# Rouslan/NTracer

Measured on AMD Instinct MI355X. Metric: Mrays/s (primary+shadow), 6-D hypercube @1920x1080, higher is better.
Workload: dtype f32

## Files before the change

### ntracer_amd/build.py

```python
import concurrent.futures
import hashlib
import os
import shutil
import subprocess
import sys

HERE = os.path.dirname(os.path.abspath(__file__))
CSRC = os.path.join(HERE, "csrc")
OBJ = os.path.join(HERE, "build")
OUT = os.path.join(HERE, "libntracer_hip.so")
DIMS = range(3, 11)
BOX_ONLY_DIMS = range(11, 25)
HDR = [os.path.join(CSRC, h) for h in ("nt_device.hpp", "nt_pixel.hpp", "nt_box.hpp", "nt_composite.hpp", "nt_resolve.hpp", "nt_query.hpp", "nt_hits.hpp", "nt_rays.hpp", "nt_lens.hpp", "nt_parallel.hpp", "nt_adaptive.hpp", "nt_ao.hpp", "nt_outline.hpp", "nt_cue.hpp", "nt_clip.hpp", "nt_boxhits.hpp", "nt_dispatch.hpp")] + \
      [os.path.join(HERE, "..", "include", "ntracer_hip.h")]
FLAGS = ["--offload-arch=gfx950", "-O3", "-std=c++17", "-ffp-contract=off", "-fPIC", "-pthread", "-fno-slp-vectorize", "-Wall",
         "-Wno-unused-function"]
EXTRA = os.environ.get("NTRACER_HIPCC_FLAGS", "").split()


def units():
    u = [("nt_api", "nt_api.cpp", []), ("nt_builder", "nt_builder.cpp", []), ("nt_launch", "nt_launch.cpp", []),
         ("nt_var", "nt_var.hip", [])]
    for n in DIMS:
        u.append(("nt_box_%d" % n, "nt_inst_box.hip", ["-DNT_INST_N=%d" % n]))
        u.append(("nt_composite_%d" % n, "nt_inst_composite.hip", ["-DNT_INST_N=%d" % n]))
        u.append(("nt_query_%d" % n, "nt_inst_query.hip", ["-DNT_INST_N=%d" % n]))
        u.append(("nt_hits_%d" % n, "nt_inst_hits.hip", ["-DNT_INST_N=%d" % n]))
        u.append(("nt_rays_%d" % n, "nt_inst_rays.hip", ["-DNT_INST_N=%d" % n]))
        u.append(("nt_adaptive_%d" % n, "nt_inst_adaptive.hip", ["-DNT_INST_N=%d" % n]))
        u.append(("nt_lens_%d" % n, "nt_inst_lens.hip", ["-DNT_INST_N=%d" % n]))
        u.append(("nt_parallel_%d" % n, "nt_inst_parallel.hip", ["-DNT_INST_N=%d" % n]))
        u.append(("nt_ao_%d" % n, "nt_inst_ao.hip", ["-DNT_INST_N=%d" % n]))
        u.append(("nt_outline_%d" % n, "nt_inst_outline.hip", ["-DNT_INST_N=%d" % n]))
        u.append(("nt_cue_%d" % n, "nt_inst_cue.hip", ["-DNT_INST_N=%d" % n]))
        u.append(("nt_boxhits_%d" % n, "nt_inst_boxhits.hip", ["-DNT_INST_N=%d" % n]))
        u.append(("nt_clip_%d" % n, "nt_inst_clip.hip", ["-DNT_INST_N=%d" % n]))
    for n in BOX_ONLY_DIMS:
        u.append(("nt_box_%d" % n, "nt_inst_box.hip", ["-DNT_INST_N=%d" % n]))
        u.append(("nt_rays_%d" % n, "nt_inst_rays.hip", ["-DNT_INST_N=%d" % n]))
        u.append(("nt_adaptive_%d" % n, "nt_inst_adaptive.hip", ["-DNT_INST_N=%d" % n]))
        u.append(("nt_boxhits_%d" % n, "nt_inst_boxhits.hip", ["-DNT_INST_N=%d" % n]))
    return u


def hipcc():
    for c in (os.environ.get("HIPCC"), shutil.which("hipcc"), "/opt/rocm/bin/hipcc"):
# ... 77 lines not shown
```

### ntracer_amd/csrc/nt_api.cpp

```cpp
#include <hip/hip_runtime_api.h>

#include <algorithm>
#include <atomic>
#include <climits>
#include <cmath>
#include <cstdarg>
#include <cstdio>
#include <cstring>
#include <cstdlib>
#include <map>
#include <memory>
#include <mutex>
#include <new>
#include <string>
#include <thread>
#include <vector>

#include "../../include/ntracer_hip.h"
#include "nt_device.hpp"

namespace {

thread_local std::string g_error;

int fail(int code, const char *fmt, ...) {
    char buf[512];
    va_list ap;
    va_start(ap, fmt);
    vsnprintf(buf, sizeof(buf), fmt, ap);
    va_end(ap);
    g_error = buf;
    return code;
}

#define HIP_TRY(expr)                                                                          \
    do {                                                                                       \
        hipError_t e_ = (expr);                                                                \
        if (e_ != hipSuccess) return fail(e_ == hipErrorOutOfMemory ? NT_E_NOMEM : NT_E_DEVICE, \
                                          "%s failed: %s", #expr, hipGetErrorString(e_));       \
    } while (0)

struct DevBuf {
    void *p = nullptr;
    size_t cap = 0;
    int ensure(size_t bytes) {
        if (bytes <= cap && p) return 0;
        if (p) { (void)hipFree(p); p = nullptr; cap = 0; }
        size_t want = std::max<size_t>(bytes, 256);
        HIP_TRY(hipMalloc(&p, want));
        cap = want;
        return 0;
    }
// ... 527 lines not shown
    }
    return NT_OK;
}

struct RenderGuard {
    nt_scene *s;
    bool held = false;
    explicit RenderGuard(nt_scene *sc) : s(sc) {}
    int acquire() {
        std::lock_guard<std::mutex> g(s->mu);
        if (s->busy) return fail(NT_E_BUSY, "the renderer is already running");
        s->busy = true;
        ++s->locked;
        held = true;
        return NT_OK;
    }
    ~RenderGuard() {
        if (held) {
            std::lock_guard<std::mutex> g(s->mu);
            s->busy = false;
            --s->locked;
        }
    }
};

struct FrameJob {
    const Format *fmt;
    Bands bands;
    void *dest_dev;
    size_t frame_stride;
    int nframes;
    const float *cam_buf;
    const float *cam_dots = nullptr;
    hipStream_t stream;
    bool stats;
    bool strict = false;
    const int *abort_word = nullptr;
    int overlapped = 0;
    bool counters_pass = false;
    bool samples_pass = false;
    int row_begin, row_count;
    float *colors_out = nullptr;
    const int *xs = nullptr, *ys = nullptr;
    int probe_count = 0;
    int view_w = 0, view_h = 0;
};

struct RenderSwitches {
    bool strict_reference, clean_normals, force_var, numerators, two_pass, tile_order, box_cull, box_interleave, box_var_rows;
    int composite_kernel, frame_major, chunk_frames;
};

int atoi_or(const char *e, int unset) { return e ? atoi(e) : unset; }

RenderSwitches read_switches() {
    RenderSwitches sw;
    sw.strict_reference = atoi_or(getenv("NTRACER_STRICT_REFERENCE"), 0) != 0;
    sw.clean_normals = atoi_or(getenv("NTRACER_CLEAN_NORMALS"), 0) != 0;
    sw.force_var = atoi_or(getenv("NTRACER_FORCE_VAR"), 0) != 0;
    sw.composite_kernel = atoi_or(getenv("NTRACER_COMPOSITE_KERNEL"), 0);
    sw.numerators = atoi_or(getenv("NTRACER_NUMERATORS"), 1) != 0;
    sw.two_pass = atoi_or(getenv("NTRACER_TWO_PASS"), 1) != 0;
    sw.tile_order = atoi_or(getenv("NTRACER_TILE_ORDER"), 1) != 0;
    sw.frame_major = atoi_or(getenv("NTRACER_FRAME_MAJOR"), 1);
    sw.chunk_frames = atoi_or(getenv("NTRACER_CHUNK_FRAMES"), INT_MAX);
    sw.box_cull = atoi_or(getenv("NTRACER_BOX_CULL"), 1) != 0;
// ... 52 lines not shown
    return NT_OK;
}

int plain_f32_format(int w, int h, Format &out) {
    static const nt_channel plain[3] = {{1.0f, 0.0f, 0.0f, 0.0f, 32, 1, {0, 0}}, {0.0f, 1.0f, 0.0f, 0.0f, 32, 1, {0, 0}}, {0.0f, 0.0f, 1.0f, 0.0f, 32, 1, {0, 0}}};
    const nt_image_format desc = {(int32_t)w, (int32_t)h, 0, 3, plain, 0};
    return parse_format(&desc, out);
}

void view_target(const nt_scene *s, int w, int h, const int *abort_word, NtTarget &tg) {
    std::memset(&tg, 0, sizeof(tg));
    fill_view(tg, s, w, h);
    tg.band_world = 1;
    tg.band_rows = NT_RENDER_CHUNK_SIZE;
    tg.row_count = h;
    tg.abort_word = abort_word;
}

FrameJob base_frame_job(const nt_scene *s, const FrameJob &job, const Format &bf, int f0, int nf, void *dest, size_t frame_bytes) {
    FrameJob bj = job;
    bj.samples_pass = true;
    bj.fmt = &bf;
    bj.bands = Bands();
    bj.bands.owned_rows = bf.height;
    bj.row_begin = 0;
    bj.row_count = bf.height;
    bj.nframes = nf;
    bj.frame_stride = frame_bytes;
    bj.dest_dev = dest;
    bj.stats = false;
    if (job.cam_buf) {
        bj.cam_buf = job.cam_buf + (size_t)f0 * 4 * s->n;
        bj.cam_dots = job.cam_dots + (size_t)f0 * 4;
    }
    return bj;
}

int checked_scratch(const nt_scene *s, DeviceState *ds, const RenderSwitches &sw, NtCompositeDev &c, long long lanes_per_block, long long &blocks,
                    long long min_blocks, int frame_stack, long long cap_bytes) {
    const long long words = ((long long)s->n_batches + s->n_triangles + s->n_solids + 31) / 32;
    const long long fwords = (long long)nt_var_frame_words(s->n) * frame_stack;
    while (blocks > min_blocks && blocks * lanes_per_block * (words + fwords) * 4 > cap_bytes) blocks /= 2;
    if (int e = ds->checked.ensure((size_t)(blocks * lanes_per_block * words * 4))) return e;
    c.checked = (uint32_t *)ds->checked.p;
    c.checked_words = (int)words;
    c.checked_lanes = (int)(blocks * lanes_per_block);
    c.alias_normals = sw.clean_normals ? 0 : 1;
    if (frame_stack > 0) {
        if (int e = ds->tframes.ensure((size_t)(blocks * lanes_per_block * fwords * 4))) return e;
        c.tframes = (float *)ds->tframes.p;
        c.tframe_count = frame_stack;
    }
    return NT_OK;
}

int numerator_scratch(const nt_scene *s, DeviceState *ds, const RenderSwitches &sw, int nframes, NtLaunchInfo &li) {
    if (s->n_batches <= 0 || !sw.numerators) return NT_OK;
    const size_t per_frame = (size_t)s->n_batches * NT_BATCH_SIZE * sizeof(float);
    const size_t frames = std::max<size_t>(1, std::min<size_t>((size_t)nframes, ((size_t)256 << 20) / per_frame));
    if (int e = ds->numer.ensure(frames * per_frame)) return e;
    li.numer_buf = (float *)ds->numer.p;
    li.numer_frames = std::max(1, std::min((int)frames, sw.chunk_frames));
    return NT_OK;
}

int hit_record_scratch(DeviceState *ds, const RenderSwitches &sw, size_t per_frame, int nframes, NtLaunchInfo &li) {
// ... 162 lines not shown
    const long long row_bytes = hi_pitch * ss;
    if (hi_pitch > INT_MAX || hi_h > INT_MAX)
        return fail(NT_E_UNSUPPORTED, "supersampling %d of a %d x %d image: the %lld x %lld samples are beyond the 2^31 - 1 bytes a sample row "
                    "and the 2^31 - 1 sample rows the kernels address", ss, f.width, f.height, hi_w, hi_h);
    if (row_bytes > cap)
        return fail(NT_E_UNSUPPORTED, "supersampling %d of a %d pixel wide image: the samples of one row (%lld bytes) do not fit the scratch "
                    "buffer of %lld MiB (nt_scene_set_supersampling_scratch_mb)", ss, f.width, row_bytes, cap >> 20);
    Format hf;
    if (int r = plain_f32_format((int)hi_w, (int)hi_h, hf)) return r;
    const long long rows_fit = std::min<long long>(cap / row_bytes, 16384);
    const int chunk_rows = (int)std::min<long long>(rows_fit, job.row_count);
    const int chunk_frames = chunk_rows < job.row_count ? 1 : (int)std::max<long long>(1, std::min<long long>(job.nframes, cap / (row_bytes * chunk_rows)));
    if (int e = ds->samples.ensure((size_t)chunk_frames * chunk_rows * row_bytes)) return e;
    NtTarget tg;
    if (int r = fill_target(s, ds, job, tg)) return r;
    for (int f0 = 0; f0 < job.nframes; f0 += chunk_frames) {
        const int nf = std::min(chunk_frames, job.nframes - f0);
        for (int r0 = 0; r0 < job.row_count; r0 += chunk_rows) {
            const int rc = std::min(chunk_rows, job.row_count - r0);
            FrameJob hj = job;
            hj.samples_pass = true;
            hj.fmt = &hf;
            hj.bands.rows = ss * job.bands.rows;
            hj.bands.compact = 1;
            hj.bands.owned_rows = ss * job.bands.owned_rows;
            hj.row_begin = ss * (job.row_begin + r0);
            hj.row_count = ss * rc;
            hj.nframes = nf;
            hj.frame_stride = (size_t)(rc * row_bytes);
            hj.dest_dev = (char *)ds->samples.p - (long long)hj.row_begin * hi_pitch;
            if (job.cam_buf) {
                hj.cam_buf = job.cam_buf + (size_t)f0 * 4 * s->n;
                hj.cam_dots = job.cam_dots + (size_t)f0 * 4;
            }
            if (int e = enqueue(s, ds, hj)) return e;
            NtTarget rt = tg;
            rt.dest = tg.dest + (long long)f0 * tg.frame_stride;
            rt.row_begin = job.row_begin + r0;
            rt.row_count = rc;
            if (int r = nt_launch_resolve(ss, job.stream, ds->samples.p, (long long)hj.frame_stride, hi_pitch, nf, rt)) return launch_failed(r);
        }
    }
    return NT_OK;
}

int rays_scene(const nt_scene *s, DeviceState *ds, const RenderSwitches &sw, bool strict, long long count, long long lpb_fixed, long long max_fixed,
               NtCompositeDev &c);

int adaptive_check(const nt_scene *s, const Bands &b, bool stats) {
    if (!s->adaptive || s->supersampling <= 1) return NT_OK;
    if (b.world > 1) return fail(NT_E_UNSUPPORTED, "row bands (band_world %d) are not available with adaptive supersampling: a pixel's contrast needs its neighbours", b.world);
    if (stats) return fail(NT_E_UNSUPPORTED, "collect_stats is not available with adaptive supersampling");
    return NT_OK;
}

int enqueue_adaptive(nt_scene *s, DeviceState *ds, const FrameJob &job, const RenderSwitches &sw, uint8_t *mask_dev, bool mask_scratch,
                     uint8_t **mask_out) {
    const bool draw = job.fmt != nullptr;
    const int ss = s->supersampling;
    const int W = draw ? job.fmt->width : job.view_w, H = draw ? job.fmt->height : job.view_h;
    if (job.bands.world > 1) return fail(NT_E_UNSUPPORTED, "row bands (band_world %d) are not available with adaptive supersampling: a pixel's contrast needs its neighbours", job.bands.world);
    if (job.stats) return fail(NT_E_UNSUPPORTED, "collect_stats is not available with adaptive supersampling");
    if (draw && (job.row_begin != 0 || job.row_count != H)) return fail(NT_E_UNSUPPORTED, "a row range is not available with adaptive supersampling");
    if (draw && job.fmt->bpp == 0) return NT_OK;
    const long long px = (long long)W * H;
    const long long cap = (long long)s->ss_scratch_mb << 20;
// ... 672 lines not shown
    if (s->outlines && s->composite && !job.colors_out && !job.samples_pass && !job.counters_pass)
        return enqueue_outlines(s, ds, job, sw, nullptr, false, nullptr);
    if (s->ao_count > 0 && s->composite && !job.colors_out && !job.samples_pass && !job.counters_pass)
        return enqueue_ao(s, ds, job, sw, nullptr, nullptr);
    if (s->box_lines && !s->composite && !job.colors_out && !job.samples_pass && !job.counters_pass)
        return enqueue_box_lines(s, ds, job, sw, nullptr, false, nullptr);
    if (s->lens) return enqueue_lens(s, ds, job, sw);
    if (s->parallel > 0.0f) return enqueue_parallel(s, ds, job, sw);
    if (s->supersampling > 1 && s->adaptive && !job.colors_out && !job.samples_pass && !job.counters_pass)
        return enqueue_adaptive(s, ds, job, sw, nullptr, false, nullptr);
    if (s->supersampling > 1 && !job.colors_out && !job.samples_pass && !job.counters_pass) return enqueue_supersampled(s, ds, job);
    if (s->composite && job.stats && !job.counters_pass && !job.colors_out) {
        if (s->n > NT_MAX_FIXED_DIM) return fail(NT_E_UNSUPPORTED, "collect_stats is not available above %d dimensions (the run-time-n kernels keep no counters)", NT_MAX_FIXED_DIM);
        if (!s->all_opaque)
            return fail(NT_E_UNSUPPORTED, "collect_stats is not available for scenes with transparent materials (their kernels keep no counters)");
        if (s->n_solids > 0 && !sw.clean_normals) {
            const size_t bytes = (size_t)job.fmt->pitch * (size_t)(job.bands.compact ? job.bands.owned_rows : job.fmt->height);
            if (int e = ds->stats_frame.ensure(std::max<size_t>(bytes, 16))) return e;
            FrameJob cj = job;
            cj.counters_pass = true;
            cj.dest_dev = ds->stats_frame.p;
            cj.frame_stride = 0;
            if (job.nframes > 1) return fail(NT_E_UNSUPPORTED, "collect_stats on a multi-frame launch is not available for scenes with Solids");
            if (int e = enqueue(s, ds, cj)) return e;
            job.stats = false;
        }
    }
    NtTarget tg;
    if (int r = fill_target(s, ds, job, tg)) return r;
    if (!job.colors_out && (tg.row_count <= 0 || tg.bpp == 0)) return NT_OK;
    NtCamera cam;
    cam.buf = job.cam_buf;
    cam.dots = job.cam_dots;
    cam.n = s->n;
    if (!job.cam_buf) pack_camera(s->n, s->origin.data(), s->axes.data(), cam.inl);
    camera_dots(s->n, s->origin.data(), s->axes.data(), cam.odots);
    NtLaunchInfo li = launch_info(s, ds, sw, job.nframes, job.stream);
    int r;
    if (s->composite) {
        NtCompositeDev c;
        if (int e = plan_composite(s, ds, job, sw, tg, cam, li, c)) return e;
        r = nt_launch_composite(li, cam, c, tg);
    } else {
        if (int e = plan_box(s, ds, job, sw, tg, li)) return e;
        r = nt_launch_box(li, cam, tg);
    }
    if (r) return launch_failed(r);
    return NT_OK;
}

int prepare_stats(DeviceState *ds, hipStream_t st, bool on) {
    if (!on) return NT_OK;
    if (int r = ds->stats.ensure(8 * sizeof(unsigned long long))) return r;
    HIP_TRY(hipMemsetAsync(ds->stats.p, 0, 8 * sizeof(unsigned long long), st));
    return NT_OK;
}

int render_checks(const nt_scene *s, const Format &f, const Bands &b, bool stats) {
    if (int r = clip_check(s, b, stats, 0, b.owned_rows, f.height)) return r;
    if (int r = cue_check(s, b, stats, 0, b.owned_rows, f.height)) return r;
    if (int r = outline_check(s, b, stats, 0, b.owned_rows, f.height)) return r;
    if (int r = ao_check(s, b, stats, 0, b.owned_rows, f.height)) return r;
    if (int r = box_lines_check(s, b, stats, 0, b.owned_rows, f.height)) return r;
    if (int r = lens_check(s, f.width, f.height, b, stats, false)) return r;
    if (int r = parallel_check(s, b, stats, false)) return r;
    return adaptive_check(s, b, stats);
// ... 1167 lines not shown
    }
    if (int r = use_stream(ds, (hipStream_t)hip_stream)) return r;
    const int n = s->n;
    const size_t cam_floats = (size_t)nframes * 4 * n + (size_t)nframes * 4;
    DeviceState::Stage *st = nullptr;
    if (int r = stage_slot(ds, cam_floats * sizeof(float), st)) return r;
    float *packed = (float *)st->host;
    pack_cameras(n, nframes, origins, axes, packed);
    if (int r = ds->cams.ensure(cam_floats * sizeof(float))) return r;
    if (int r = nt_launch_upload(hip_stream, packed, (float *)ds->cams.p, (int)cam_floats)) return launch_failed(r);
    HIP_TRY(hipEventRecord(st->done, (hipStream_t)hip_stream));
    st->in_flight = true;
    if (int r = prepare_stats(ds, (hipStream_t)hip_stream, stats)) return r;
    if (stats) { s->have_stats = false; s->stats_device = ds->device; }
    FrameJob job = render_job(f, b, dest_dev, frame_stride, nframes, (hipStream_t)hip_stream, stats, opts, true);
    job.cam_buf = (const float *)ds->cams.p;
    job.cam_dots = job.cam_buf + (size_t)nframes * 4 * s->n;
    return enqueue(s, ds, job);
}

struct nt_camera_table {
    int n = 0, nframes = 0, device = -1;
    float *dev = nullptr;
};

nt_camera_table_t *nt_camera_table_create(int dimension, int nframes, const float *origins, const float *axes, int device) {
    if (dimension < 3 || dimension > NT_MAX_DIM || nframes < 1 || nframes > 65535 || !origins || !axes) {
        fail(NT_E_INVALID, "invalid camera table arguments");
        return nullptr;
    }
    int dev;
    if (pick_device(nullptr, device, dev)) return nullptr;
    const int n = dimension;
    const size_t cam_floats = (size_t)nframes * 4 * n + (size_t)nframes * 4;
    std::vector<float> packed(cam_floats);
    pack_cameras(n, nframes, origins, axes, packed.data());
    void *p = nullptr;
    if (hipMalloc(&p, cam_floats * sizeof(float)) != hipSuccess) { fail(NT_E_NOMEM, "hipMalloc failed for the camera table"); return nullptr; }
    if (hipMemcpy(p, packed.data(), cam_floats * sizeof(float), hipMemcpyHostToDevice) != hipSuccess) {
        (void)hipFree(p);
        fail(NT_E_DEVICE, "camera table upload failed");
        return nullptr;
    }
    nt_camera_table *t = new (std::nothrow) nt_camera_table();
    if (!t) { (void)hipFree(p); fail(NT_E_NOMEM, "out of memory"); return nullptr; }
    t->n = n; t->nframes = nframes; t->device = dev; t->dev = (float *)p;
    return t;
}

void nt_camera_table_destroy(nt_camera_table_t *t) {
    if (!t) return;
    if (t->dev && hipSetDevice(t->device) == hipSuccess) { (void)hipDeviceSynchronize(); (void)hipFree(t->dev); }
    delete t;
}

int nt_camera_table_frames(const nt_camera_table_t *t) { return t ? t->nframes : fail(NT_E_INVALID, "table is NULL"); }

int nt_render_table_device(nt_scene_t *s, void *dest_dev, size_t frame_stride, const nt_camera_table_t *table, int first, int count,
                           const nt_image_format *fmt, const nt_render_opts *opts, void *hip_stream) {
    if (!s || !dest_dev || !table) return fail(NT_E_INVALID, "NULL argument");
    if (table->n != s->n) return fail(NT_E_INVALID, "the camera table is for %d dimensions, the scene has %d", table->n, s->n);
    if (first < 0 || count < 1 || first > table->nframes - count) return fail(NT_E_INVALID, "frames %d..%d are not in a table of %d", first, first + count - 1, table->nframes);
    Format f;
    if (int r = parse_format(fmt, f)) return r;
    Bands b;
    if (int r = parse_bands(opts, f.height, b)) return r;
    if (frame_stride < required_len(f, b)) return fail(NT_E_INVALID, "frame_stride is smaller than one frame");
    if (int r = check_renderable(s)) return r;
    std::lock_guard<std::mutex> g(s->mu);
    if (s->busy) return fail(NT_E_BUSY, "the renderer is already running");
    const bool stats = opts && opts->collect_stats;
    if (int r = render_checks(s, f, b, stats)) return r;
    DeviceState *ds;
    if (int r = scene_on_device(s, opts, -1, ds, table->device, "render")) return r;
    if (int r = use_stream(ds, (hipStream_t)hip_stream)) return r;
    if (int r = prepare_stats(ds, (hipStream_t)hip_stream, stats)) return r;
    if (stats) { s->have_stats = false; s->stats_device = ds->device; }
    FrameJob job = render_job(f, b, dest_dev, frame_stride, count, (hipStream_t)hip_stream, stats, opts, true);
    job.cam_buf = table->dev + (size_t)first * 4 * table->n;
    job.cam_dots = table->dev + (size_t)table->nframes * 4 * table->n + (size_t)first * 4;
    return enqueue(s, ds, job);
}

namespace {
int mask_validate(const nt_scene *s, int width, int height, const void *mask, const nt_render_opts *opts) {
    if (!s || !mask) return fail(NT_E_INVALID, "NULL argument");
    if (width < 1 || height < 1) return fail(NT_E_INVALID, "invalid view size");
    if (int r = clip_refuses(s, "the adaptive mask")) return r;
    if (!s->adaptive) return fail(NT_E_INVALID, "the adaptive threshold is off (nt_scene_set_adaptive_supersampling)");
    if (opts && opts->band_world > 1)
        return fail(NT_E_UNSUPPORTED, "the adaptive mask is of the whole image: row bands (band_world %d) are not available", opts->band_world);
    if (opts && opts->collect_stats) return fail(NT_E_UNSUPPORTED, "the adaptive mask keeps no counters: collect_stats is not available");
    if (s->lens || s->parallel > 0.0f) return fail(NT_E_UNSUPPORTED, "the adaptive mask is not available while a lens or the parallel projection is set");
    return check_renderable(s);
}
}

int nt_adaptive_mask(nt_scene_t *s, int width, int height, uint8_t *mask, long long *flagged, const nt_render_opts *opts) {
    if (int r = mask_validate(s, width, height, mask, opts)) return r;
    RenderGuard guard(s);
    if (int r = guard.acquire()) return r;
    DeviceState *ds;
    if (int r = scene_on_device(s, opts, -1, ds)) return r;
    if (int r = use_own_stream(ds)) return r;
    const FrameJob job = view_job(width, height, ds->stream, opts, false);
    uint8_t *mask_dev = nullptr;
    if (int r = enqueue_adaptive(s, ds, job, read_switches(), nullptr, true, &mask_dev)) { (void)hipStreamSynchronize(ds->stream); return r; }
    int count = 0;
    HIP_TRY(hipMemcpyAsync(mask, mask_dev, (size_t)width * height, hipMemcpyDeviceToHost, ds->stream));
    HIP_TRY(hipMemcpyAsync(&count, ds->refine_count.p, sizeof(int), hipMemcpyDeviceToHost, ds->stream));
    HIP_TRY(hipStreamSynchronize(ds->stream));
    if (flagged) *flagged = count;
    return NT_OK;
// ... 317 lines not shown
```

### ntracer_amd/csrc/nt_box.hpp

```cpp
#pragma once
#include <type_traits>
#include "nt_pixel.hpp"

namespace {

__device__ __forceinline__ bool box_may_hit(int n, const float *dots, float sx, float sy, float sq) {
    const float osq = dots[0];
    const float ov = fmaf(-dots[2], sy, fmaf(dots[1], sx, dots[3]));
    const float rad2 = (float)n * (1.0f + NT_FUZZ) * (1.0f + NT_FUZZ) * 1.001f;
#ifdef NT_EXP_SKIP_SLABS
    return false;
#else
    return !((osq - rad2) * sq > ov * ov * 1.0001f);
#endif
}

__device__ __forceinline__ void box_background(float in, float &r, float &g, float &b) {
    if (in > 0.0f) { r = in; g = in; b = in; }
    else { r = 0.0f; g = -in; b = -in; }
}

template <int N>
__device__ __forceinline__ void box_color(const float (&o)[N], const float (&dir)[N], bool maybe, float &r, float &g, float &b) {
    bool done = false;
    float shade = 0.0f;

    {
        float num[N];
        bool pre[N];
        float aK = 0.0f, bK = 1.0f, oK = 0.0f;
        bool any = false;
#pragma unroll
        for (int i = 0; i < N; ++i) {
            const float di = dir[i];
            const float s = di < 0.0f ? 1.0f : -1.0f;
// ... 13 lines not shown
                bool ok = tie && dist > 0.0f;
#pragma unroll
                for (int j = 0; j < N; ++j) {
                    if (j != i) {
                        const float p = dir[j] * dist + o[j];
                        ok = ok && !(fabsf(p) > (1.0f + NT_FUZZ));
                    }
                }
                if (ok) {
                    done = true;
                    if (dist >= FLT_MAX) shade = -1.0f;
                    else {
                        const float sine = di * (di < 0.0f ? 1.0f : -1.0f);
                        shade = sine <= 0.0f ? -sine : 0.0f;
                    }
                }
            }
        }
    }
    if (done && shade >= 0.0f) {
        r = shade * 1.0f;
        g = shade * 0.5f;
        b = shade * 0.5f;
    } else {
        box_background(dir[0], r, g, b);
    }
}

#ifndef NT_BOX_INLINE_MAX_N
#define NT_BOX_INLINE_MAX_N 8
#endif
#ifndef NT_BOX_SETS_MAX_N
#define NT_BOX_SETS_MAX_N NT_BOX_INLINE_MAX_N
#endif
#ifndef NT_BOX_MARGIN
#define NT_BOX_MARGIN 1e-5f
#endif
template <int N>
__device__ __forceinline__ void box_classify(const float (&o)[N], const float (&v)[N], float m, bool maybe, bool &hit, bool &unclear,
                                             float &x, float (&near)[N], float &tn, float &vK) {
    float tn2 = -INFINITY;
    tn = -INFINITY;
    vK = 0.0f;
    float tnp = -INFINITY, tfp = INFINITY;
    const float m1p = 1.0f + m;
#pragma unroll
    for (int j = 0; j < N; ++j) {
        const float inv = __builtin_amdgcn_rcpf(v[j]);
        const float c0 = -o[j] * inv;
        const float nr = c0 - fabsf(inv);
        near[j] = nr;
        tnp = fmaxf(tnp, fmaf(-fabsf(inv), m1p, c0));
        tfp = fminf(tfp, fmaf(fabsf(inv), m1p, c0));
        const bool later = nr > tn;
        tn2 = __builtin_amdgcn_fmed3f(tn, tn2, nr);
        vK = later ? v[j] : vK;
        tn = fmaxf(tn, nr);
    }
    const bool miss = tnp > tfp || tfp < 0.0f;
    const float c = 1.0f - m;
    float sum = 0.0f;
#pragma unroll
    for (int j = 0; j < N; ++j) sum = sum + fmaxf(fabsf(fmaf(v[j], tn, o[j])), c);
    const bool inside = sum - (float)N * c <= 1.5f * m;
    const bool sole = (tn - tn2) * fabsf(vK) > m;
    const bool front = tn > 1e-3f && tn < 1e30f;
    hit = maybe && !miss && inside && sole && front;
    unclear = maybe && !miss && !hit;
#ifdef NT_EXP_NOUNCLEAR
    unclear = false;
#endif
    x = hit ? vK : v[0];
}

__device__ __forceinline__ float nt_vmax(float a, float b) { float r; asm("v_max_f32 %0, %1, %2" : "=v"(r) : "v"(a), "v"(b)); return r; }
__device__ __forceinline__ float nt_vmin(float a, float b) { float r; asm("v_min_f32 %0, %1, %2" : "=v"(r) : "v"(a), "v"(b)); return r; }
__device__ __forceinline__ float nt_vmax3(float a, float b, float c) { float r; asm("v_max3_f32 %0, %1, %2, %3" : "=v"(r) : "v"(a), "v"(b), "v"(c)); return r; }
__device__ __forceinline__ float nt_vmin3(float a, float b, float c) { float r; asm("v_min3_f32 %0, %1, %2, %3" : "=v"(r) : "v"(a), "v"(b), "v"(c)); return r; }
__device__ __forceinline__ float nt_vmed3(float a, float b, float c) { float r; asm("v_med3_f32 %0, %1, %2, %3" : "=v"(r) : "v"(a), "v"(b), "v"(c)); return r; }
__device__ __forceinline__ float nt_vmax_abs(float a, float b) { float r; asm("v_max_f32 %0, |%1|, %2" : "=v"(r) : "v"(a), "v"(b)); return r; }
__device__ __forceinline__ float nt_vmax3_abs(float a, float b, float c) { float r; asm("v_max3_f32 %0, %1, |%2|, |%3|" : "=v"(r) : "v"(a), "v"(b), "v"(c)); return r; }
__device__ __forceinline__ float nt_vmin_abs(float a, float b) { float r; asm("v_min_f32 %0, |%1|, %2" : "=v"(r) : "v"(a), "v"(b)); return r; }

#ifndef NT_BOX_TIE_SHORTCUT
#define NT_BOX_TIE_SHORTCUT 1
#endif
#ifndef NT_BOX_TIE_SHORTCUT_MIN_N
#define NT_BOX_TIE_SHORTCUT_MIN_N 6
#endif
#ifndef NT_BOX_TIE_SHORTCUT_MAX_N
#define NT_BOX_TIE_SHORTCUT_MAX_N 8
#endif
#ifndef NT_BOX_TIE_SURE_MAX_ORIGIN
#define NT_BOX_TIE_SURE_MAX_ORIGIN 4.5f
#endif
#ifndef NT_BOX_TIE_SHORTCUT_MIN_WAVES
#define NT_BOX_TIE_SHORTCUT_MIN_WAVES 32768
#endif
#define NT_BOX_SETS_SURE 0x01000000u
template <int N>
constexpr bool nt_box_tie_shortcut() { return NT_BOX_TIE_SHORTCUT != 0 && N >= NT_BOX_TIE_SHORTCUT_MIN_N && N <= NT_BOX_TIE_SHORTCUT_MAX_N && N <= NT_BOX_SETS_MAX_N; }

#ifndef NT_BOX_CLASSIFY_SETS_MIN_N
#define NT_BOX_CLASSIFY_SETS_MIN_N 6
#endif
#ifndef NT_BOX_CLASSIFY_SETS_MAX_N
#define NT_BOX_CLASSIFY_SETS_MAX_N 7
#endif
template <int N>
__device__ __forceinline__ void box_classify_sets(const float (&o)[N], const float (&v)[N], float m, uint32_t sets, bool &hit, bool &unclear,
                                                  float &x) {
    float tn = -INFINITY, tn2 = -INFINITY, vK = 0.0f;
    float tnp = -INFINITY, tfp = INFINITY;
    const float m1p = 1.0f + m;
#pragma unroll
    for (int j = 0; j < N; ++j) {
        if (((sets >> (10 + j)) & 1u) != 0u) {
            const float inv = __builtin_amdgcn_rcpf(v[j]);
            const float c0 = -o[j] * inv;
            tfp = nt_vmin(tfp, fmaf(fabsf(inv), m1p, c0));
            if (((sets >> j) & 1u) != 0u) {
                const float nr = c0 - fabsf(inv);
                tnp = nt_vmax(tnp, fmaf(-fabsf(inv), m1p, c0));
                const bool later = nr > tn;
                tn2 = nt_vmed3(tn, tn2, nr);
                vK = later ? v[j] : vK;
                tn = nt_vmax(tn, nr);
            }
        }
    }
    const bool miss = tnp > tfp || tfp < 0.0f;
    const float c = 1.0f - m;
// ... 644 lines not shown
    __shared__ uint32_t s_sets[SETS_LDS ? LDS_N : 1];
    __shared__ int s_abort;
    uint32_t lane_cs = 0u;
    const int tid = (int)threadIdx.x;
    const int lane = tid & 63;
    const int wv = __builtin_amdgcn_readfirstlane(tid >> 6);
#ifdef NT_EXP_TRACE
    const unsigned long long trace_t0 = wall_clock64();
    unsigned trace_rows = 0u;
    unsigned long long trace_t1 = 0ull;
#endif
    const unsigned nframes = gridDim.z - (unsigned)tg.lead_frames;
    unsigned frame = blockIdx.z;
    if (tg.lead_frames > 0) {
        const unsigned cols = gridDim.x, q = cols / 4u;
        const bool middle = blockIdx.x >= q && blockIdx.x < cols - q;
        if (!middle) frame -= (unsigned)tg.lead_frames;
        if (frame >= nframes) return;
    }
    float org[N], right[N], up[N], fwd[N], dir[N];
    load_camera<N>(cam, frame, org, right, up, fwd);
    float margin = fabsf(org[0]);
#pragma unroll
    for (int j = 1; j < N; ++j) margin = fmaxf(margin, fabsf(org[j]));
    margin = NT_BOX_MARGIN * (1.0f + margin);
    float dots[4];
    if (cam.buf) {
        const float *dp = cam.dots + (size_t)frame * 4;
        dots[0] = dp[0]; dots[1] = dp[1]; dots[2] = dp[2]; dots[3] = dp[3];
    } else {
        dots[0] = cam.odots[0]; dots[1] = cam.odots[1]; dots[2] = cam.odots[2]; dots[3] = cam.odots[3];
    }
    const int tile_row0 = (int)blockIdx.y * WAVES * R;
    if (REG || wv == (int)((blockIdx.x + blockIdx.y + frame) % (unsigned)WAVES)) {
        if (tg.abort_word != nullptr) {
            const bool ab = nt_aborted(tg);
            if constexpr (REG) { if (ab) return; }
            else { if (lane == 0) s_abort = ab ? 1 : 0; }
        }
        uint32_t code = 0u;
        uint32_t row_sets = 0u;
        const int trow = tg.row_il > 0 ? ((int)blockIdx.y * WAVES + lane / R) + tg.row_il * (lane % R) : tile_row0 + lane;
        if (lane < WAVES * R && trow < tg.row_count) {
            const int orow = tg.row_begin + trow;
            const int y = nt_image_row(tg, orow);
            if (y < tg.height) {
                const unsigned long long cs = box_stretch_code2<N, (N <= NT_BOX_SETS_MAX_N), TIE>(org, right, up, fwd, tg, y, (int)blockIdx.x);
                code = (uint32_t)cs;
                row_sets = (uint32_t)(cs >> 32);
            }
        }
        if constexpr (REG) {
            lane_cs = (SETS_LDS ? row_sets & SETS_MASK : 0u) | (code << 20);
        } else {
            if (SETS_LDS) s_sets[lane] = row_sets;
            {
                const unsigned long long m0 = __builtin_amdgcn_ballot_w64(code == 0u), m1 = __builtin_amdgcn_ballot_w64(code >= 1u && code <= 13u),
                                         m2 = __builtin_amdgcn_ballot_w64(code == 15u), m3 = __builtin_amdgcn_ballot_w64(code == 14u);
                if (lane == 0) {
                    s_rows[0] = m0;
                    s_rows[1] = m1;
                    s_rows[2] = m2;
                    s_rows[3] = m3;
                }
            }
            uint32_t packed = code << (4 * (lane & 7));
            packed |= (uint32_t)__shfl_xor((int)packed, 1, 64);
            packed |= (uint32_t)__shfl_xor((int)packed, 2, 64);
            packed |= (uint32_t)__shfl_xor((int)packed, 4, 64);
            if ((lane & 7) == 0) {
                const int grp = lane >> 3;
                const int slot = R == 8 ? 2 * grp : grp;
                s_code[slot] = packed;
                if (R == 8) s_code[slot + 1] = 0u;
            }
        }
// ... 293 lines not shown
                const int rr = nt_low_bit(redo_bits);
                nt_drop_low_bit(redo_bits, rr);
                const int mrow = il > 0 ? hfirst + il * rr : row0 + rr;
                atomicOr(tg.redo + ((size_t)frame * tg.row_count + mrow) * tg.redo_words + (blockIdx.x >> 5), 1u << (blockIdx.x & 31));
            }
        }
        }
    }
#ifdef NT_EXP_TRACE
    if (lane == 0) {
        unsigned long long *tr = reinterpret_cast<unsigned long long *>(tg.dest + (long long)nframes * tg.frame_stride) +
                                 ((((size_t)frame * gridDim.y + blockIdx.y) * gridDim.x + blockIdx.x) * WAVES + wv) * 4;
        tr[0] = trace_t0;
        tr[1] = wall_clock64();
        tr[2] = (unsigned long long)__builtin_amdgcn_s_getreg(4 | (31 << 11)) | ((unsigned long long)__builtin_amdgcn_s_getreg(20 | (31 << 11)) << 32);
        tr[3] = (unsigned long long)trace_rows | ((trace_t1 - trace_t0) << 32);
    }
#endif
#undef NT_ROW_LOAD
#undef NT_ROW_OFF
#undef NT_ROW_PTR
#undef NT_GROUP_PTR
#undef NT_LANE_OFF
#undef NT_CLEAR_BIT
#undef NT_SET_BIT
#undef NT_RED_OF
}

template <int N>
int launch_box_fixed(const NtLaunchInfo &li, const NtCamera &cam, const NtTarget &tg_in) {
    NtCameraFixed cf;
    cf.buf = cam.buf;
    cf.dots = cam.dots;
    for (int k = 0; k < 4; ++k) cf.odots[k] = cam.odots[k];
    cf.n = N;
    for (int k = 0; k < 4 * N; ++k) cf.inl[k] = cam.inl[k];
    NtTarget tg = tg_in;
    dim3 grid;
    grid_for(tg, 64, tg.colors_out ? 4 : 4 * NT_BOXROWS, li.nframes, grid);
    tg.cull = nullptr;
    tg.redo = nullptr;
    tg.cull_words = 0;
    tg.redo_words = 0;
    const bool fmt_rgb = tg.plain_bits != 0u && tg.plain_bits <= 10u && tg.bpp == 4 && tg.aligned4;
    const bool fmt_f32 = tg.plain_f32[0] >= 0 && tg.bpp == 12 && tg.aligned4;
    if (li.cull_buf && tg.rowtab && !tg.colors_out && (fmt_rgb || fmt_f32) && li.cull_clean) {
        hipStream_t st = (hipStream_t)li.stream;
        NtBoxTileGeom geom;
        geom.rows = li.tile_rows;
        geom.waves = li.tile_waves;
        const bool r64 = geom.rows == 64, r16 = geom.rows == 16;
        const int wpb = geom.waves;
        const int tile_rows = geom.rows * geom.waves;
        dim3 tgrid((unsigned)((tg.width + 63) / 64), (unsigned)((tg.row_count + tile_rows - 1) / tile_rows), (unsigned)li.nframes);
        tg.redo_words = ((tg.width + 63) / 64 + 31) / 32;
        tg.redo = li.cull_buf;
        tg.lead_frames = li.nframes >= 8 ? (li.nframes < 96 ? li.nframes : 96) : 0;
        if (tg.row_il > 0) tg.lead_frames = li.nframes >= 32 ? 16 : 0;
        if ((long long)li.nframes + tg.lead_frames > 65535) tg.lead_frames = 0;
        tgrid.z += (unsigned)tg.lead_frames;
        if (fmt_rgb) {
            bool tie = false;
            if constexpr (nt_box_tie_shortcut<N>()) tie = r64 && (unsigned long long)tgrid.x * tgrid.y * (unsigned)li.nframes >= (unsigned long long)NT_BOX_TIE_SHORTCUT_MIN_WAVES;
            if (tie) {
                if constexpr (nt_box_tie_shortcut<N>()) hipLaunchKernelGGL((box_tile_kernel<N, false, 64, 1, true>), tgrid, dim3(64), 0, st, cf, tg);
            } else if (r64) hipLaunchKernelGGL((box_tile_kernel<N, false, 64, 1>), tgrid, dim3(64), 0, st, cf, tg);
// ... 33 lines not shown
```

### ntracer_amd/csrc/nt_device.hpp

```cpp
#pragma once
#include <stdint.h>

#define NT_DEV_MAX_DIM 64
#define NT_DEV_MAX_FIXED 10
#define NT_DEV_MAX_FIXED_BOX 24
#define NT_DEV_BATCH 4
#define NT_DEV_MAX_REFLECT 16

#define NT_FUZZ (1.1920928955078125e-07f * 10.0f)
#define NT_LIGHT_THRESHOLD (1.0f / 512.0f)

struct NtChanDev {
    float f_r, f_g, f_b, f_c;
    uint32_t bits;
    uint32_t tfloat;
    uint32_t offset;
    uint32_t maxval;
};

#define NT_PACK_GENERIC 0
#define NT_PACK_WORD32 1
#define NT_PACK_WORD64 2

struct NtTarget {
    uint8_t *dest;
    long long frame_stride;
    const NtChanDev *chans;
    int nchannels, bpp, reversed, pitch;
    int pack_mode;
    uint32_t plain_bits, plain_maxval, plain_mul[3];
    uint32_t plain_sel;
    int plain_f32[3];
    int width, height;
    float half_w, half_h, fovI;
    int band_rank, band_world, band_rows, compact;
    int row_begin, row_count;
    int aligned4;
    float *colors_out;
    const int *probe_xs, *probe_ys;
    int probe_count;
    const void *hits;
    const uint32_t *cull;
    int cull_words;
    uint32_t *redo;
    int redo_words;
    const void *rowtab;
    int row_il;
    const int *abort_word;
    int lead_frames;
};

struct NtCamera {
    const float *buf;
    const float *dots;
    int n;
    float odots[4];
    float inl[4 * NT_DEV_MAX_DIM];
};
struct NtCameraFixed {
    const float *buf;
    const float *dots;
    int n;
    float odots[4];
    float inl[4 * NT_DEV_MAX_FIXED_BOX];
};

struct NtNode {
    float split;
    int axis;
    int left;
    int right;
};

struct NtCompositeDev {
    const NtNode *nodes;
    const int *items;
    const float *batch_recs;
    const int *batch_mats;
    const float *tri_recs;
    const int *tri_mats;
    const float *solid_recs;
    const int *solid_types;
    const int *solid_mats;
    const float *materials;
    const float *aabb;
    int rec_stride;
    int root;
    int stack_depth;
    int shadows, camera_light, max_reflect_depth, bg_axis;
    float ambient[3], bg1[3], bg2[3], bg3[3];
    int n_point_lights;
    const float *pl_pos;
    const float *pl_color;
    int n_global_lights;
// ... 221 lines not shown
```

Baseline: 1.102 million.

## Precompute per-frame hypercube screen-x span to skip empty column strips

On the host, the change computes a conservative screen-x interval covering the projected (margin-padded) hypercube for each frame in the camera table. It stores the interval alongside the camera data. In the box kernel, a 64-column strip whose x range lies outside the interval skips the per-row classification. The intent is to avoid ray-box work for columns that cannot hit the box, at the cost of extra host-side vertex enumeration and the risk of a non-conservative span dropping hits.

```diff
diff --git a/ntracer_amd/build.py b/ntracer_amd/build.py
--- a/ntracer_amd/build.py
+++ b/ntracer_amd/build.py
@@ -11,7 +11,7 @@
 OUT = os.path.join(HERE, "libntracer_hip.so")
 DIMS = range(3, 11)
 BOX_ONLY_DIMS = range(11, 25)
-HDR = [os.path.join(CSRC, h) for h in ("nt_device.hpp", "nt_pixel.hpp", "nt_box.hpp", "nt_composite.hpp", "nt_resolve.hpp", "nt_query.hpp", "nt_hits.hpp", "nt_rays.hpp", "nt_lens.hpp", "nt_parallel.hpp", "nt_adaptive.hpp", "nt_ao.hpp", "nt_outline.hpp", "nt_cue.hpp", "nt_clip.hpp", "nt_boxhits.hpp", "nt_dispatch.hpp")] + \
+HDR = [os.path.join(CSRC, h) for h in ("nt_device.hpp", "nt_pixel.hpp", "nt_box.hpp", "nt_box_span.hpp", "nt_composite.hpp", "nt_resolve.hpp", "nt_query.hpp", "nt_hits.hpp", "nt_rays.hpp", "nt_lens.hpp", "nt_parallel.hpp", "nt_adaptive.hpp", "nt_ao.hpp", "nt_outline.hpp", "nt_cue.hpp", "nt_clip.hpp", "nt_boxhits.hpp", "nt_dispatch.hpp")] + \
       [os.path.join(HERE, "..", "include", "ntracer_hip.h")]
 FLAGS = ["--offload-arch=gfx950", "-O3", "-std=c++17", "-ffp-contract=off", "-fPIC", "-pthread", "-fno-slp-vectorize", "-Wall",
          "-Wno-unused-function"]
diff --git a/ntracer_amd/csrc/nt_api.cpp b/ntracer_amd/csrc/nt_api.cpp
--- a/ntracer_amd/csrc/nt_api.cpp
+++ b/ntracer_amd/csrc/nt_api.cpp
@@ -18,6 +18,7 @@
 
 #include "../../include/ntracer_hip.h"
 #include "nt_device.hpp"
+#include "nt_box_span.hpp"
 
 namespace {
 
@@ -611,6 +612,7 @@
     int nframes;
     const float *cam_buf;
     const float *cam_dots = nullptr;
+    const float *cam_span = nullptr;
     hipStream_t stream;
     bool stats;
     bool strict = false;
@@ -729,6 +731,7 @@
     if (job.cam_buf) {
         bj.cam_buf = job.cam_buf + (size_t)f0 * 4 * s->n;
         bj.cam_dots = job.cam_dots + (size_t)f0 * 4;
+        if (job.cam_span) bj.cam_span = job.cam_span + (size_t)f0 * 2;
     }
     return bj;
 }
@@ -957,6 +960,7 @@
             if (job.cam_buf) {
                 hj.cam_buf = job.cam_buf + (size_t)f0 * 4 * s->n;
                 hj.cam_dots = job.cam_dots + (size_t)f0 * 4;
+                if (job.cam_span) hj.cam_span = job.cam_span + (size_t)f0 * 2;
             }
             if (int e = enqueue(s, ds, hj)) return e;
             NtTarget rt = tg;
@@ -1695,6 +1699,7 @@
     NtCamera cam;
     cam.buf = job.cam_buf;
     cam.dots = job.cam_dots;
+    cam.span = job.cam_buf ? job.cam_span : nullptr;
     cam.n = s->n;
     if (!job.cam_buf) pack_camera(s->n, s->origin.data(), s->axes.data(), cam.inl);
     camera_dots(s->n, s->origin.data(), s->axes.data(), cam.odots);
@@ -2928,9 +2933,16 @@
     int dev;
     if (pick_device(nullptr, device, dev)) return nullptr;
     const int n = dimension;
-    const size_t cam_floats = (size_t)nframes * 4 * n + (size_t)nframes * 4;
+    const size_t span_at = (size_t)nframes * 4 * n + (size_t)nframes * 4;
+    const size_t cam_floats = span_at + (size_t)nframes * 2;
     std::vector<float> packed(cam_floats);
     pack_cameras(n, nframes, origins, axes, packed.data());
+    for (int f = 0; f < nframes; ++f) {
+        const float *o = origins + (size_t)f * n, *ax = axes + (size_t)f * n * n;
+        const NtBoxSpan sp = nt_box_strip_span(n, o, ax, ax + n, ax + 2 * n);
+        packed[span_at + 2 * (size_t)f] = sp.lo;
+        packed[span_at + 2 * (size_t)f + 1] = sp.hi;
+    }
     void *p = nullptr;
     if (hipMalloc(&p, cam_floats * sizeof(float)) != hipSuccess) { fail(NT_E_NOMEM, "hipMalloc failed for the camera table"); return nullptr; }
     if (hipMemcpy(p, packed.data(), cam_floats * sizeof(float), hipMemcpyHostToDevice) != hipSuccess) {
@@ -2975,6 +2987,7 @@
     FrameJob job = render_job(f, b, dest_dev, frame_stride, count, (hipStream_t)hip_stream, stats, opts, true);
     job.cam_buf = table->dev + (size_t)first * 4 * table->n;
     job.cam_dots = table->dev + (size_t)table->nframes * 4 * table->n + (size_t)first * 4;
+    job.cam_span = table->dev + (size_t)table->nframes * (4 * table->n + 4) + (size_t)first * 2;
     return enqueue(s, ds, job);
 }
 
diff --git a/ntracer_amd/csrc/nt_box.hpp b/ntracer_amd/csrc/nt_box.hpp
--- a/ntracer_amd/csrc/nt_box.hpp
+++ b/ntracer_amd/csrc/nt_box.hpp
@@ -1,6 +1,7 @@
 #pragma once
 #include <type_traits>
 #include "nt_pixel.hpp"
+#include "nt_box_span.hpp"
 
 namespace {
 
@@ -80,9 +81,6 @@
 #endif
 #ifndef NT_BOX_SETS_MAX_N
 #define NT_BOX_SETS_MAX_N NT_BOX_INLINE_MAX_N
-#endif
-#ifndef NT_BOX_MARGIN
-#define NT_BOX_MARGIN 1e-5f
 #endif
 template <int N>
 __device__ __forceinline__ void box_classify(const float (&o)[N], const float (&v)[N], float m, bool maybe, bool &hit, bool &unclear,
@@ -146,6 +144,9 @@
 #define NT_BOX_TIE_SHORTCUT_MIN_WAVES 32768
 #endif
 #define NT_BOX_SETS_SURE 0x01000000u
+#ifndef NT_BOX_STRIP_SPAN
+#define NT_BOX_STRIP_SPAN 1
+#endif
 template <int N>
 constexpr bool nt_box_tie_shortcut() { return NT_BOX_TIE_SHORTCUT != 0 && N >= NT_BOX_TIE_SHORTCUT_MIN_N && N <= NT_BOX_TIE_SHORTCUT_MAX_N && N <= NT_BOX_SETS_MAX_N; }
 
@@ -856,6 +857,17 @@
         dots[0] = cam.odots[0]; dots[1] = cam.odots[1]; dots[2] = cam.odots[2]; dots[3] = cam.odots[3];
     }
     const int tile_row0 = (int)blockIdx.y * WAVES * R;
+    bool strip_out = false;
+    if constexpr (NT_BOX_STRIP_SPAN != 0 && N <= NT_BOX_SPAN_MAX_N) {
+      if (cam.span != nullptr) {
+        const float *sp = cam.span + (size_t)frame * 2;
+        const float span_lo = sp[0], span_hi = sp[1];
+        const int x_first = (int)blockIdx.x * 64;
+        const int x_last = x_first + 63 < tg.width ? x_first + 63 : tg.width - 1;
+        const float sx_a = tg.fovI * ((float)x_first - tg.half_w), sx_b = tg.fovI * ((float)x_last - tg.half_w);
+        strip_out = fmaxf(sx_a, sx_b) < span_lo || fminf(sx_a, sx_b) > span_hi;
+      }
+    }
     if (REG || wv == (int)((blockIdx.x + blockIdx.y + frame) % (unsigned)WAVES)) {
         if (tg.abort_word != nullptr) {
             const bool ab = nt_aborted(tg);
@@ -865,7 +877,7 @@
         uint32_t code = 0u;
         uint32_t row_sets = 0u;
         const int trow = tg.row_il > 0 ? ((int)blockIdx.y * WAVES + lane / R) + tg.row_il * (lane % R) : tile_row0 + lane;
-        if (lane < WAVES * R && trow < tg.row_count) {
+        if (!strip_out && lane < WAVES * R && trow < tg.row_count) {
             const int orow = tg.row_begin + trow;
             const int y = nt_image_row(tg, orow);
             if (y < tg.height) {
@@ -1225,6 +1237,7 @@
     NtCameraFixed cf;
     cf.buf = cam.buf;
     cf.dots = cam.dots;
+    cf.span = cam.buf ? cam.span : nullptr;
     for (int k = 0; k < 4; ++k) cf.odots[k] = cam.odots[k];
     cf.n = N;
     for (int k = 0; k < 4 * N; ++k) cf.inl[k] = cam.inl[k];
diff --git a/ntracer_amd/csrc/nt_box_span.hpp b/ntracer_amd/csrc/nt_box_span.hpp
--- /dev/null
+++ b/ntracer_amd/csrc/nt_box_span.hpp
@@ -0,0 +1,106 @@
+#pragma once
+#include <cmath>
+#include <limits>
+
+#ifndef NT_BOX_SPAN_MAX_N
+#define NT_BOX_SPAN_MAX_N 10
+#endif
+#define NT_BOX_SPAN_SLACK 1e-4
+#define NT_BOX_SPAN_TAU_MIN 1e-3
+#ifndef NT_BOX_MARGIN
+#define NT_BOX_MARGIN 1e-5f
+#endif
+
+struct NtBoxSpan { float lo, hi; };
+
+static inline NtBoxSpan nt_box_strip_span(int n, const float *origin, const float *right, const float *up, const float *fwd) {
+    const float inf = std::numeric_limits<float>::infinity();
+    const NtBoxSpan none = {-inf, inf}, empty = {inf, -inf};
+    if (n < 3 || n > NT_BOX_SPAN_MAX_N || !origin || !right || !up || !fwd) return none;
+    float omax = 0.0f;
+    for (int j = 0; j < n; ++j) {
+        if (!std::isfinite(origin[j]) || !std::isfinite(right[j]) || !std::isfinite(up[j]) || !std::isfinite(fwd[j])) return none;
+        omax = std::fmax(omax, std::fabs(origin[j]));
+    }
+    const float mf = NT_BOX_MARGIN * (1.0f + omax);
+    const float hf = 1.0f + 2.0f * mf + 1e-3f;
+    const double h = (double)hf;
+    double c[NT_BOX_SPAN_MAX_N][3], L[NT_BOX_SPAN_MAX_N], U[NT_BOX_SPAN_MAX_N], len[NT_BOX_SPAN_MAX_N];
+    for (int j = 0; j < n; ++j) {
+        c[j][0] = (double)fwd[j];
+        c[j][1] = (double)right[j];
+        c[j][2] = -(double)up[j];
+        L[j] = -h - (double)origin[j];
+        U[j] = h - (double)origin[j];
+        len[j] = std::sqrt(c[j][0] * c[j][0] + c[j][1] * c[j][1] + c[j][2] * c[j][2]);
+    }
+    auto det3 = [&](int i, int j, int k) {
+        return c[i][0] * (c[j][1] * c[k][2] - c[j][2] * c[k][1]) - c[i][1] * (c[j][0] * c[k][2] - c[j][2] * c[k][0]) + c[i][2] * (c[j][0] * c[k][1] - c[j][1] * c[k][0]);
+    };
+    int ks[NT_BOX_SPAN_MAX_N], nk = 0;
+    for (int q = 0; q < n; ++q) {
+        bool doubtful = false;
+        for (int a = 0; a < nk && !doubtful; ++a)
+            for (int b = a + 1; b < nk && !doubtful; ++b) {
+                const double rel = std::fabs(det3(ks[a], ks[b], q)) / (len[ks[a]] * len[ks[b]] * len[q]);
+                doubtful = rel > 0.0 && rel < 1e-6;
+            }
+        if (!doubtful) ks[nk++] = q;
+    }
+    double gram[3][3] = {{0, 0, 0}, {0, 0, 0}, {0, 0, 0}};
+    for (int a = 0; a < nk; ++a)
+        for (int p = 0; p < 3; ++p)
+            for (int q = 0; q < 3; ++q) gram[p][q] += c[ks[a]][p] * c[ks[a]][q];
+    const double gdet = gram[0][0] * (gram[1][1] * gram[2][2] - gram[1][2] * gram[2][1]) - gram[0][1] * (gram[1][0] * gram[2][2] - gram[1][2] * gram[2][0]) +
+                        gram[0][2] * (gram[1][0] * gram[2][1] - gram[1][1] * gram[2][0]);
+    const double gscale = gram[0][0] * gram[1][1] * gram[2][2];
+    const double gmax = std::fmax(gram[0][0], std::fmax(gram[1][1], gram[2][2])), gmin = std::fmin(gram[0][0], std::fmin(gram[1][1], gram[2][2]));
+    if (!(gscale > 0.0) || !(gmin >= 1e-6 * gmax) || !(gdet > 1e-6 * gscale)) return none;
+    const double tol = 1e-7 * (h + (double)omax);
+    double tau_min = INFINITY, tau_max = -INFINITY, lo = INFINITY, hi = -INFINITY;
+    int nverts = 0;
+    for (int ai = 0; ai < nk; ++ai)
+        for (int aj = ai + 1; aj < nk; ++aj) {
+            const int i = ks[ai], j = ks[aj];
+            const double x0 = c[i][1] * c[j][2] - c[i][2] * c[j][1], x1 = c[i][2] * c[j][0] - c[i][0] * c[j][2], x2 = c[i][0] * c[j][1] - c[i][1] * c[j][0];
+            for (int ak = aj + 1; ak < nk; ++ak) {
+                const int k = ks[ak];
+                const double det = x0 * c[k][0] + x1 * c[k][1] + x2 * c[k][2];
+                const double rel = std::fabs(det) / (len[i] * len[j] * len[k]);
+                if (!(rel >= 1e-9)) continue;
+                const double y0 = c[j][1] * c[k][2] - c[j][2] * c[k][1], y1 = c[j][2] * c[k][0] - c[j][0] * c[k][2], y2 = c[j][0] * c[k][1] - c[j][1] * c[k][0];
+                const double z0 = c[k][1] * c[i][2] - c[k][2] * c[i][1], z1 = c[k][2] * c[i][0] - c[k][0] * c[i][2], z2 = c[k][0] * c[i][1] - c[k][1] * c[i][0];
+                const double inv = 1.0 / det;
+                for (int s = 0; s < 8; ++s) {
+                    const double di = (s & 1) ? U[i] : L[i], dj = (s & 2) ? U[j] : L[j], dk = (s & 4) ? U[k] : L[k];
+                    const double tau = (di * y0 + dj * z0 + dk * x0) * inv, a = (di * y1 + dj * z1 + dk * x1) * inv, b = (di * y2 + dj * z2 + dk * x2) * inv;
+                    bool inside = true;
+                    for (int aq = 0; aq < nk && inside; ++aq) {
+                        const int q = ks[aq];
+                        if (q == i || q == j || q == k) continue;
+                        const double v = c[q][0] * tau + c[q][1] * a + c[q][2] * b;
+                        inside = v >= L[q] - tol && v <= U[q] + tol;
+                    }
+                    if (!inside) continue;
+                    ++nverts;
+                    tau_min = std::fmin(tau_min, tau);
+                    tau_max = std::fmax(tau_max, tau);
+                    if (tau > 0.0) {
+                        const double sx = a / tau;
+                        lo = std::fmin(lo, sx);
+                        hi = std::fmax(hi, sx);
+                    }
+                }
+            }
+        }
+    if (nverts == 0 || tau_max <= -NT_BOX_SPAN_TAU_MIN) return empty;
+    if (!(tau_min > NT_BOX_SPAN_TAU_MIN) || !std::isfinite(lo) || !std::isfinite(hi)) return none;
+    lo -= NT_BOX_SPAN_SLACK * (1.0 + std::fabs(lo));
+    hi += NT_BOX_SPAN_SLACK * (1.0 + std::fabs(hi));
+    NtBoxSpan r;
+    r.lo = (float)lo;
+    if ((double)r.lo > lo) r.lo = std::nextafterf(r.lo, -inf);
+    r.hi = (float)hi;
+    if ((double)r.hi < hi) r.hi = std::nextafterf(r.hi, inf);
+    return r;
+}
diff --git a/ntracer_amd/csrc/nt_device.hpp b/ntracer_amd/csrc/nt_device.hpp
--- a/ntracer_amd/csrc/nt_device.hpp
+++ b/ntracer_amd/csrc/nt_device.hpp
@@ -53,6 +53,7 @@
 struct NtCamera {
     const float *buf;
     const float *dots;
+    const float *span = nullptr;
     int n;
     float odots[4];
     float inl[4 * NT_DEV_MAX_DIM];
@@ -60,6 +61,7 @@
 struct NtCameraFixed {
     const float *buf;
     const float *dots;
+    const float *span = nullptr;
     int n;
     float odots[4];
     float inl[4 * NT_DEV_MAX_FIXED_BOX];
```

Result: faster. 1.118 million, median of 6 (+1.4%).
